# DaveStrickland/AstroPhotography

Measured on AMD Instinct MI355X. Metric: Mpixels/sec calibrate+sigma-clip-stack, higher is better.
Workload: dtype f32; 1 GPU; C2: 64x4096x4096 f32 per GPU, fused bias/dark/flat + 3-sigma maxiters-5 median-centred clipped mean; frames_per_gpu=64, frames_total=64, height=4096, width=4096, parallelism=single GPU

## Files before the change

### astrophotography_amd/csrc/stack_calibrate.h

```cpp
#pragma once
#include "stack_sort.h"

namespace apgpu_stack {

using namespace apgpu;

struct StackParams {
    const void *frames;
    const float *bias, *dark, *nflat, *exp_ratio, *pedestal;
    const uint8_t *pixmask;
    float *mean, *median, *std;
    void *moments;
    int32_t *count;
    int64_t P;
    int64_t stride;
    double sl2, su2;
    int N;
    int still_biased;
    int center;
    int dev;
    int maxiters;
    int moments64;
    double *mean64, *std64;
    int single_kernel;
// ... 90 lines not shown
    }
}

template <int NP>
__device__ __forceinline__ void stage_commit(const StackParams &prm, FrameScalars<NP> &fs, float e, float ped)
{
    const int t = threadIdx.x;
    if (t < NP) {
        fs.e[t] = e;
        fs.ped[t] = ped;
        fs.pad[t] = t < prm.N ? -__builtin_inff() : __builtin_inff();
    }
    __syncthreads();
}

template <int NP>
__device__ __forceinline__ void stage_frame_scalars(const StackParams &prm, FrameScalars<NP> &fs)
{
    for (int t = threadIdx.x; t < NP; t += blockDim.x) {
        const int ff = t < prm.N ? t : prm.N - 1;
        fs.e[t] = prm.exp_ratio ? prm.exp_ratio[ff] : 0.f;
        fs.ped[t] = prm.pedestal ? prm.pedestal[ff] : 0.f;
        fs.pad[t] = t < prm.N ? -__builtin_inff() : __builtin_inff();
    }
    __syncthreads();
}

#ifndef APGPU_PIN_RAGGED_F32
#define APGPU_PIN_RAGGED_F32 0
#endif
template <int NP, typename RawT, bool FULL, int F0 = 0, int CNT = NP, int MINN = 0, int NSTATIC = 0>
__device__ __forceinline__ void load_raw(const StackParams &prm, int64_t base, int lane, RawT (&raw)[CNT])
{
    const RawT *fb = static_cast<const RawT *>(prm.frames) + base + (int64_t)F0 * prm.stride;
    int nframes = NSTATIC > 0 ? NSTATIC : prm.N;
    if constexpr (!FULL && NSTATIC == 0) asm volatile("" : "+s"(nframes));
#pragma unroll
    for (int f = 0; f < CNT; f++) {
        constexpr bool SKIP = !FULL && MINN < NP;
        if (!SKIP || F0 + f < MINN || F0 + f < nframes) raw[f] = fb[lane];
        else raw[f] = RawT(0);
        if (FULL || (SKIP && F0 + f + 1 < MINN) || F0 + f + 1 < nframes) fb += prm.stride;
        if ((f & 7) == 7) __builtin_amdgcn_sched_barrier(0);
    }
    if constexpr ((sizeof(RawT) == 2 || APGPU_PIN_RAGGED_F32) && !FULL && MINN < NP && NSTATIC == 0) {
#pragma unroll
        for (int f = 0; f < CNT; f++) asm volatile("" : "+v"(raw[f]));
    }
}

typedef float v2f __attribute__((ext_vector_type(2)));

template <int NP, typename RawT, bool HAS_PED, int F0 = 0, int CNT = NP, bool RANGE_GUARD = true, int MINN = NP, bool UNI_E = false,
          bool E_DIRECT = false>
__device__ __forceinline__ bool calibrate_fast(const FrameScalars<NP> &fs, const RawT (&raw)[CNT], float b, float D, float nf,
                                               bool dodiv, float (&v)[NP], int nframes = NP, int plo = 0, const float *eg = nullptr)
{
    const float nfe = dodiv ? nf : 1.0f;
    const float y = __fdiv_rn(1.0f, nfe);
    const float yl = recip_low(nfe, y);
    const float anf = fabsf(nfe);
    const bool nf_ok = (anf >= 0x1p-40f && anf <= 0x1p40f);
    float mx = 0.f, mn = __builtin_inff();
    if constexpr (NP >= 2) {
        v2f acc = {0.f, 0.f};
        const v2f b2 = {b, b}, D2 = {D, D}, nf2 = {-nfe, -nfe}, y2 = {y, y}, yl2 = {yl, yl}, zero2 = {0.f, 0.f};
        float e0 = 0.f;
        if constexpr (UNI_E) {
            if constexpr (E_DIRECT) e0 = ((const float __attribute__((address_space(4))) *)(uintptr_t)eg)[0];
            else e0 = fs.e[0];
        }
        const float ds0 = e0 * D;
        const v2f ds_uni = {ds0, ds0};
#pragma unroll
        for (int g = 0; g < CNT; g += 2) {
            const int f = F0 + g;
            if ((f & ~7) >= MINN && (f & ~7) >= nframes) continue;
            v2f x = {to_f32(raw[g]), to_f32(raw[g + 1])};
            if constexpr (HAS_PED) {
                const v2f ped = {fs.ped[f], fs.ped[f + 1]};
                x = x + ped;
            }
            x = x - b2;
            v2f ds = ds_uni;
            if constexpr (UNI_E) {
            } else if constexpr (E_DIRECT) {
                typedef const float __attribute__((address_space(4))) cfloat;
                const cfloat *ec = (const cfloat *)(uintptr_t)eg;
                const int f0 = (f < MINN || f < nframes) ? f : nframes - 1;
                const int f1 = (f + 1 < MINN || f + 1 < nframes) ? f + 1 : nframes - 1;
                const v2f e2 = {ec[f0], ec[f1]};
                ds = e2 * D2;
            } else {
                const v2f e2 = {fs.e[f], fs.e[f + 1]};
                ds = e2 * D2;
            }
            x = x - ds;
            const v2f q0 = __builtin_elementwise_fma(x, y2, x * yl2);
            const v2f r0 = __builtin_elementwise_fma(nf2, q0, x);
            const v2f q = __builtin_elementwise_fma(r0, y2, q0);
            v[f] = q.x;
            v[f + 1] = q.y;
            acc = __builtin_elementwise_fma(q, zero2, acc);
            if constexpr (RANGE_GUARD) {
                mx = fmaxf(fmaxf(mx, fabsf(q.x)), fabsf(q.y));
                mn = fminf(fminf(mn, fabsf(q.x)), fabsf(q.y));
            }
        }
        if constexpr (MINN < NP) {
#pragma unroll
            for (int g = 0; g < CNT; g++)
                if (F0 + g >= MINN && F0 + g >= nframes)
                    v[F0 + g] = (F0 + g < nframes + plo) ? -__builtin_inff() : __builtin_inff();
        }
        const bool range_ok = !RANGE_GUARD || !dodiv || (mx < 0x1p50f && mn > 0x1p-50f);
        return nf_ok && range_ok && (acc.x == 0.f) && (acc.y == 0.f);
    } else {
        float x = to_f32(raw[0]);
        if constexpr (HAS_PED) x = x + fs.ped[0];
        x = x - b;
        const float ds = (E_DIRECT ? eg[0] : fs.e[0]) * D;
        x = x - ds;
        const float q = div_by_recip(x, nfe, y, yl);
        v[0] = q;
        const float acc = __builtin_fmaf(q, 0.0f, 0.0f);
        const bool range_ok = !dodiv || (fabsf(q) < 0x1p50f && fabsf(q) > 0x1p-50f);
        return nf_ok && range_ok && (acc == 0.f);
    }
}

template <int LO, int NP>
__device__ __forceinline__ float uniform_pick(const float (&v)[NP], int idx)
{
    if constexpr (LO >= NP - 1) return v[NP - 1];
    else {
        if (idx <= LO) return v[LO];
        return uniform_pick<LO + 1, NP>(v, idx);
    }
}

template <int NP, int MINN = NP>
__device__ __forceinline__ bool range_ok_sorted(const float (&v)[NP], bool dodiv, int nvalid = NP, int plo = 0)
{
    float lo = v[0];
    float hi;
    if constexpr (MINN >= NP) hi = v[NP - 1];
    else {
        if (plo > 0) lo = uniform_pick<0, NP>(v, plo);
        hi = uniform_pick<(MINN > 0 ? MINN - 1 : 0), NP>(v, plo + __builtin_amdgcn_readfirstlane(nvalid) - 1);
    }
    const bool big_ok = fmaxf(fabsf(lo), fabsf(hi)) < 0x1p50f;
    const bool one_sign = lo > 0x1p-50f || hi < -0x1p-50f;
    bool small_ok = one_sign;
    if (wave_any(dodiv && !one_sign)) {
        float mn = __builtin_inff();
        if constexpr (NP >= 2) {
#pragma unroll
            for (int i = 0; i < NP; i += 2) mn = fminf(fminf(mn, fabsf(v[i])), fabsf(v[i + 1]));
        } else {
            mn = fabsf(v[0]);
        }
        small_ok = mn > 0x1p-50f;
    }
    return !dodiv || (big_ok && small_ok);
}

template <int NP, typename RawT>
struct EarlyLoads {
    RawT raw[NP];
    float b, d, nf;
    bool skip;
};

template <int NP, typename RawT, bool CALIB, bool FULL, int MINN, int NSTATIC = 0>
__device__ __forceinline__ void issue_early_loads(const StackParams &prm, int64_t base, int lane, EarlyLoads<NP, RawT> &L)
{
    const int64_t p = base + lane;
    L.b = 0.f; L.d = 0.f; L.nf = 1.f;
    if constexpr (CALIB) {
        L.b = prm.bias[p];
        L.d = prm.dark[p];
        if (prm.nflat) L.nf = prm.nflat[p];
    }
    L.skip = prm.pixmask && prm.pixmask[p];
    __builtin_amdgcn_sched_barrier(0);
    load_raw<NP, RawT, FULL, 0, NP, MINN, NSTATIC>(prm, base, lane, L.raw);
}

template <int NP>
__device__ __forceinline__ bool exposures_uniform(const FrameScalars<NP> &fs)
{
    bool same = true;
    for (int t = threadIdx.x & 63; t < NP; t += 64) same = same && (fs.e[t] == fs.e[0]);
    return wave_all(same);
}

template <int NP>
__device__ __forceinline__ bool ratios_uniform(const float *eg, int nframes)
{
    typedef const float __attribute__((address_space(4))) cfloat;
    const cfloat *ec = (const cfloat *)(uintptr_t)eg;
    const int e0 = __builtin_amdgcn_readfirstlane(__float_as_int(ec[0]));
    bool same = true;
#pragma unroll
    for (int f = 1; f < NP; f++) same = same && (f >= nframes || __builtin_amdgcn_readfirstlane(__float_as_int(ec[f < nframes ? f : 0])) == e0);
    return same;
}

struct ColumnCtx {
    float b, D, nf;
    bool dodiv, skip;
    bool range_pending;
};

template <int NP, typename RawT, bool CALIB, bool FINITE_ONLY, bool FULL, int NRAW>
__device__ __forceinline__ int load_column_exact(const StackParams &prm, const FrameScalars<NP> &fs, int64_t p, const ColumnCtx &cx,
                                                 const RawT (&raw)[NRAW], float (&v)[NP], int plo = 0)
{
    const int N = prm.N;
    int n = 0;
    const RawT *fp = static_cast<const RawT *>(prm.frames) + p;
    int nleft = N;
    asm volatile("" : "+s"(nleft));
#pragma unroll
    for (int f = 0; f < NP; f++) {
        float x;
        if constexpr (CALIB) {
            x = to_f32(*fp);
            if (FULL || f + 1 < nleft) fp += prm.stride;
        } else {
            x = to_f32(raw[f < NRAW ? f : 0]);
        }
        if constexpr (CALIB) {
            typedef const float __attribute__((address_space(4))) cfloat;
            const int ff = (FULL || f < N) ? f : N - 1;
            const float e = prm.exp_ratio ? ((const cfloat *)(uintptr_t)prm.exp_ratio)[ff] : 0.f;
            const float ped = prm.pedestal ? ((const cfloat *)(uintptr_t)prm.pedestal)[ff] : 0.f;
            if (ped != 0.f) x = x + ped;
            x = x - cx.b;
            const float ds = e * cx.D;
            x = x - ds;
            if (cx.dodiv) x = __fdiv_rn(x, cx.nf);
        }
        bool ok;
        if constexpr (FINITE_ONLY) ok = fabsf(x) < __builtin_inff();
        else ok = (x == x);
        ok = ok && (FULL || f < N) && !cx.skip;
        n += ok ? 1 : 0;
        v[f] = ok ? x : __builtin_inff();
        if (!FULL && f >= N && f < N + plo) v[f] = -__builtin_inff();
    }
    return n;
}

template <int NP, typename RawT, bool CALIB, bool FINITE_ONLY, bool FULL, int MINN = padded_minn(NP, FULL), bool FORCE_HALVES = false, bool PRE = false>
__device__ __forceinline__ int load_column(const StackParams &prm, const FrameScalars<NP> &fs, int64_t base, int lane,
                                           float (&v)[NP], ColumnCtx &cx, int plo = 0, const EarlyLoads<NP, RawT> &pre = EarlyLoads<NP, RawT>())
{
    const int N = prm.N;
// ... 125 lines not shown
```

### astrophotography_amd/csrc/stack_kernels.h

```cpp
#pragma once
#include "stack_reduce.h"

namespace apgpu_stack {

using namespace apgpu;

#ifndef APGPU_LEAN_MIN_BLOCKS
#define APGPU_LEAN_MIN_BLOCKS 3
#endif
#ifndef APGPU_PLUS_MIN_BLOCKS
#define APGPU_PLUS_MIN_BLOCKS 3
#endif
#ifndef APGPU_WIDE_MIN_BLOCKS
#define APGPU_WIDE_MIN_BLOCKS 2
#endif
#ifndef APGPU_PADDED_MIN_BLOCKS
#define APGPU_PADDED_MIN_BLOCKS 3
#endif

constexpr int kRedoSegs = 256;
constexpr int kWsLine = 16;
constexpr int kWsStats = kRedoSegs * kWsLine;
constexpr int kWsCall = kWsStats + 16;
constexpr int kWsMadCount = 8, kWsMadMode = 10, kMadSample = 16;
// ... 322 lines not shown
#pragma unroll
                for (int i = 0; i < NP; i++) {
                    if (i >= nslots) continue;
                    const double dd = widen(v[i]) - mean64;
                    const bool in = (i >= T && i < NP - T) || ((i >= a) && (i < b));
                    const double d = in ? dd : 0.0;
                    q1 = fma(d, d, q1);
                }
                if (good) ko->std[p] = (float)sqrt(q1 > 0.0 ? q1 / (double)(b - a) : 0.0);
            }
        }
    }
}

template <int NP, typename RawT, bool CALIB, bool FULL = true, int PADS = 0, bool PLUS = false>
__global__ __launch_bounds__(256, NP <= 64 ? APGPU_FAST_MIN_BLOCKS : ((FULL || PADS > 0 || NP <= 96) ? 3 : 2)) void stack_fast_kernel(const StackParams prm)
{
    static_assert(PADS == 0 || (!FULL && PADS <= NP - prev_slots(NP)), "static pads: a padded stack");
    constexpr int MINN = fast_kernel_minn(NP, FULL);
    constexpr int PLO = PADS > 0 ? (PADS >> 1) : -1, PHI = PADS > 0 ? PADS - (PADS >> 1) : -1;
    static_assert(fast_kernel_slots(NP), "the fast kernel is the float32 fast path");
    static_assert(CALIB || sizeof(RawT) == 4, "unfused stacks: float32 frames");
    constexpr int T = !CALIB ? (NP >= 20 ? 8 : 6) : fast_kernel_tail(NP, FULL);
    constexpr bool HALVES = CALIB && NP >= 104;
    const int64_t base = (int64_t)blockIdx.x * 256;
    const int lane = threadIdx.x;
    const int64_t p = base + lane;
    __shared__ FrameScalars<NP> fs;
    const int N = FULL ? NP : (PADS > 0 ? NP - PADS : prm.N);
    const int plo = FULL ? 0 : (NP - N) >> 1, phi = FULL ? 0 : NP - N - plo;
    const bool alert = fast_kernel_alert();
    if (fast_block_bails<256>(alert, prm.redo)) {
        give_blocks_up<256>();
        return;
    }
    bool good = false;
    if (base + 256 <= prm.P) {
        float v[NP];
        bool dodiv = false;
        int nonfin = 0;
        if constexpr (HALVES) {
            constexpr int HN = NP / 2, NS = PADS > 0 ? NP - PADS : 0;
            const float b = prm.bias[p];
            const float D = prm.still_biased ? prm.dark[p] - b : prm.dark[p];
            float nf = 1.f;
            if (prm.nflat) {
                nf = prm.nflat[p];
                dodiv = (nf != 0.f);
            }
            good = !(prm.pixmask && prm.pixmask[p]);
            __builtin_amdgcn_sched_barrier(0);
            RawT half[HN];
            load_raw<NP, RawT, FULL, 0, HN, MINN, NS>(prm, base, lane, half);
            good = calibrate_fast<NP, RawT, false, 0, HN, false, MINN, false, true>(fs, half, b, D, nf, dodiv, v, N, plo, prm.exp_ratio) && good;
            load_raw<NP, RawT, FULL, HN, HN, MINN, NS>(prm, base, lane, half);
            good = calibrate_fast<NP, RawT, false, HN, HN, false, MINN, false, true>(fs, half, b, D, nf, dodiv, v, N, plo, prm.exp_ratio) && good;
        }
        EarlyLoads<NP, RawT> L;
        if constexpr (!HALVES) {
            issue_early_loads<NP, RawT, CALIB, FULL, MINN, (PADS > 0 ? NP - PADS : 0)>(prm, base, lane, L);
            good = !L.skip;
        }
        if constexpr (HALVES) {
        } else if constexpr (CALIB) {
            const float b = L.b;
            const float D = prm.still_biased ? L.d - b : L.d;
            float nf = 1.f;
            if (prm.nflat) {
                nf = L.nf;
                dodiv = (nf != 0.f);
            }
            good = calibrate_fast<NP, RawT, false, 0, NP, false, MINN, false, true>(fs, L.raw, b, D, nf, dodiv, v, N, plo, prm.exp_ratio) && good;
        } else {
#pragma unroll
            for (int f = 0; f < NP; f++) {
                if (FULL || f < MINN || f < N) {
                    const float x = L.raw[f];
                    v[f] = fabsf(x) < __builtin_inff() ? x : __builtin_inff();
                } else {
                    v[f] = (f < N + plo) ? -__builtin_inff() : __builtin_inff();
                }
            }
        }
#ifdef APGPU_VARIANT_STRIP
        if (wave_any(good)) {
            if (APGPU_VARIANT_STRIP == 1) {
                sort_column<NP, T>(v);
                if constexpr (CALIB) good = good && range_ok_sorted<NP, MINN>(v, dodiv, N, plo);
            }
            float acc[4] = {good ? 0.f : 1.f, 0.f, 0.f, 0.f};
#pragma unroll
            for (int i = 0; i < NP; i++) acc[i & 3] += v[i];
            if (prm.mean) prm.mean[p] = (acc[0] + acc[1]) + (acc[2] + acc[3]);
        }
        __shared__ char geometry[40 * 1024];
        if (prm.N < 0) geometry[lane] = 1;
        return;
#endif
        if (wave_any(good)) {
            sort_column<NP, T>(v);
            if constexpr (CALIB) good = good && range_ok_sorted<NP, MINN>(v, dodiv, N, plo);
            else {
#pragma unroll
                for (int k = 1; k <= T; k++) nonfin += (v[NP - k] == __builtin_inff()) ? 1 : 0;
                good = good && nonfin < T;
            }
            if (wave_any(good)) finish_fast_column<NP, T, CALIB, PLO, PHI, PLUS>(v, good, p, plo, CALIB ? phi : nonfin);
        }
    }
    fast_blocks_done<256>(alert, prm.redo);
    redo_push(!good && p < late_params()->P, p, alert);
}

template <int NP, typename RawT, bool CALIB, bool FULL>
__global__ __launch_bounds__(256) void stack_median_kernel(const StackParams prm)
{
    const int64_t base = (int64_t)blockIdx.x * blockDim.x;
    const int lane = threadIdx.x;
    const int64_t p = base + lane;
    __shared__ FrameScalars<NP> fs;
    if (needs_staging<CALIB, FULL, NP>(prm)) stage_frame_scalars<NP>(prm, fs);
    if (p >= prm.P) return;
    float v[NP];
    const int n = load_sorted_column<NP, RawT, CALIB, false, FULL>(prm, fs, base, lane, v);
    const float m1 = pick_at<NP>(v, (n - 1) >> 1);
    const float m2 = pick_at<NP>(v, n >> 1);
    const double med = ((double)m1 + (double)m2) / 2.0;
    if (prm.median) prm.median[p] = n > 0 ? (float)med : __builtin_nanf("");
    if (prm.count) prm.count[p] = n;
}

template <bool CALIB>
__device__ __forceinline__ float calibrate_exact_u16(unsigned raw, float b, float D, float e, float nf, bool dodiv)
{
    float x = (float)raw;
    if constexpr (CALIB) {
        x = x - b;
        const float ds = e * D;
        x = x - ds;
        if (dodiv) x = __fdiv_rn(x, nf);
    }
    return x;
}

template <int NP, bool CALIB, bool FULL>
__global__ __launch_bounds__(256) void stack_median_u16_kernel(const StackParams prm)
{
    __shared__ FrameScalars<NP> fs;
    const int lane = threadIdx.x;
    bool monotone = true;
    if constexpr (CALIB) {
        stage_frame_scalars<NP>(prm, fs);
        const bool differs = lane < NP && (!(fs.e[lane] == fs.e[0]) || fs.ped[lane] != 0.f);
        monotone = !__syncthreads_or(differs);
    } else if constexpr (!FULL) {
        stage_frame_scalars<NP>(prm, fs);
    }
    const int N = prm.N;
    if (monotone) {
        const int64_t p2 = ((int64_t)blockIdx.x * 256 + lane) * 2;
        if (p2 >= prm.P) return;
// ... 32 lines not shown
                nn[0] = n2.x; nn[1] = n2.y;
                dodiv[0] = n2.x != 0.f;
                dodiv[1] = n2.y != 0.f;
            }
        }
        float med[2];
        int cnt[2];
#pragma unroll
        for (int h = 0; h < 2; h++) {
            const unsigned r1 = (m1 >> (16 * h)) & 0xffffu, r2 = (m2 >> (16 * h)) & 0xffffu;
            const float c1 = calibrate_exact_u16<CALIB>(r1, bb[h], dd[h], e, nn[h], dodiv[h]);
            const float c2 = calibrate_exact_u16<CALIB>(r2, bb[h], dd[h], e, nn[h], dodiv[h]);
            const bool skip = prm.pixmask && prm.pixmask[p2 + h];
            const bool any = (c1 == c1) && (c2 == c2) && !skip;
            cnt[h] = any ? N : 0;
            med[h] = any ? (float)(((double)c1 + (double)c2) / 2.0) : __builtin_nanf("");
        }
        if (prm.median) *reinterpret_cast<float2 *>(prm.median + p2) = make_float2(med[0], med[1]);
        if (prm.count) *reinterpret_cast<int2 *>(prm.count + p2) = make_int2(cnt[0], cnt[1]);
    } else {
#pragma unroll 1
        for (int half = 0; half < 2; half++) {
            const int64_t base = ((int64_t)blockIdx.x * 2 + half) * 256;
            const int64_t p = base + lane;
            if (p >= prm.P) break;
            float v[NP];
            StackParams q = prm;
            asm volatile("" : "+s"(q.N));
            const int n = load_sorted_column<NP, uint16_t, CALIB, false, FULL, NP>(q, fs, base, lane, v);
            const float m1 = pick_at<NP>(v, (n - 1) >> 1);
            const float m2 = pick_at<NP>(v, n >> 1);
            const double med = ((double)m1 + (double)m2) / 2.0;
            if (prm.median) prm.median[p] = n > 0 ? (float)med : __builtin_nanf("");
            if (prm.count) prm.count[p] = n;
        }
    }
}

template <int NP, bool CALIB, bool FULL, int T, int MINN, int PLO = -1, int PHI = -1>
__device__ __forceinline__ bool fast_raw_column(const FrameScalars<NP> &fs, const uint32_t (&cur)[NP / 2], float b, float D, float nf,
                                                bool dv, bool masked, const float *eg, int64_t p, int N, int plo, int phi)
{
    float v[NP];
    bool good = !masked;
    {
        float rawf[NP];
#pragma unroll
        for (int k = 0; k < NP / 2; k++) {
            rawf[2 * k] = (float)(cur[k] & 0xffffu);
            rawf[2 * k + 1] = (float)(cur[k] >> 16);
        }
        if constexpr (CALIB) {
            const bool increasing = (fabsf(b) < __builtin_inff()) && (fabsf(D) < __builtin_inff()) && (!dv || (nf > 0.f && nf < __builtin_inff()));
            good = calibrate_fast<NP, float, false, 0, NP, false, NP, true, true>(fs, rawf, b, D, nf, dv, v, NP, 0, eg) && increasing && good;
        } else {
#pragma unroll
            for (int f = 0; f < NP; f++) v[f] = rawf[f];
        }
    }
    if constexpr (!FULL) {
#pragma unroll
        for (int i = 0; i < NP; i++) {
            if (i < NP - MINN && i < plo) v[i] = -__builtin_inff();
            if (i >= MINN && i >= NP - phi) v[i] = __builtin_inff();
        }
    }
    if constexpr (CALIB) good = good && range_ok_sorted<NP, (MINN < NP ? MINN : 0)>(v, dv, N, plo);
    if (wave_any(good)) finish_fast_column<NP, T, true, PLO, PHI>(v, good, p, plo, phi);
    return good;
}

constexpr bool pairs_padded_slots(int np) { return fast32_possible_padded(np, padded_minn(np, false)) || np == 104; }

template <int NP, bool CALIB, bool FULL, int PADS = 0>
__global__ __launch_bounds__(256, NP <= 80 ? APGPU_FAST_MIN_BLOCKS : (NP <= 104 ? 3 : 2)) void stack_fast_u16_pairs_kernel(const StackParams prm)
{
    static_assert(PADS == 0 || (!FULL && PADS <= NP - padded_minn(NP, false)), "static pads: a padded stack");
    constexpr int MINN = padded_minn(NP, FULL);
    constexpr int PLO = PADS > 0 ? (PADS >> 1) : -1, PHI = PADS > 0 ? PADS - (PADS >> 1) : -1;
    static_assert(FULL ? fast_kernel_slots(NP) : pairs_padded_slots(NP), "the fast kernel is the float32 fast path");
    constexpr int T = FULL ? kFastTail : fast_tail_padded(NP);
    constexpr int HP = NP / 2;
    __shared__ uint32_t parked[HP][256];
    __shared__ FrameScalars<NP> fs;
    const int lane = threadIdx.x;
    const int N = FULL ? NP : (PADS > 0 ? NP - PADS : prm.N);
    const int plo = FULL ? 0 : (NP - N) >> 1, phi = FULL ? 0 : NP - N - plo;
    const int64_t p2 = ((int64_t)blockIdx.x * 256 + lane) * 2;
    bool good0 = false, good1 = false;
    const bool tile_ok = ((int64_t)blockIdx.x + 1) * 512 <= prm.P;
    const bool alert = fast_kernel_alert();
    bool give_up = fast_block_bails<512>(alert, prm.redo);
    if constexpr (CALIB) give_up = give_up || !ratios_uniform<NP>(prm.exp_ratio, N);
    if (give_up) {
        give_blocks_up<512>();
        return;
    }
    if (tile_ok) {
        float bb[2] = {0.f, 0.f}, dd[2] = {0.f, 0.f}, nn[2] = {1.f, 1.f};
        bool dodiv[2] = {false, false};
        bool skip[2] = {false, false};
        if constexpr (CALIB) {
            const float2 b2 = *reinterpret_cast<const float2 *>(prm.bias + p2);
            const float2 d2 = *reinterpret_cast<const float2 *>(prm.dark + p2);
            bb[0] = b2.x; bb[1] = b2.y;
            dd[0] = prm.still_biased ? d2.x - b2.x : d2.x;
            dd[1] = prm.still_biased ? d2.y - b2.y : d2.y;
            if (prm.nflat) {
                const float2 n2 = *reinterpret_cast<const float2 *>(prm.nflat + p2);
                nn[0] = n2.x; nn[1] = n2.y;
                dodiv[0] = n2.x != 0.f;
                dodiv[1] = n2.y != 0.f;
            }
        }
        if (prm.pixmask) {
            skip[0] = prm.pixmask[p2] != 0;
            skip[1] = prm.pixmask[p2 + 1] != 0;
        }
        __builtin_amdgcn_sched_barrier(0);
        uint32_t w[NP];
// ... 280 lines not shown
```

### astrophotography_amd/csrc/stack_sort.h

```cpp
#pragma once
#include "common.h"

#include <utility>

namespace apgpu_stack {

using namespace apgpu;


#ifdef APGPU_PROFILE_SECTIONS
#define APGPU_MARK(name) do { __builtin_amdgcn_sched_barrier(0); asm volatile("; APGPU_SECTION " name); __builtin_amdgcn_sched_barrier(0); } while (0)
#else
#define APGPU_MARK(name) asm volatile("; APGPU_SECTION " name)
#endif

__device__ __forceinline__ bool wave_any(bool p) { return __builtin_amdgcn_ballot_w64(p) != 0; }
__device__ __forceinline__ bool wave_all(bool p) { return __builtin_amdgcn_ballot_w64(!p) == 0; }

struct CE {
    unsigned char a, b;
};

template <int NP>
struct Net {
// ... 24 lines not shown
                        net.ce[c].b = (unsigned char)(i + j + k);
                        c++;
                    }
            }
    net.n = c;
    return net;
}

template <int NP, int P0, int T>
constexpr Net<NP> make_pruned_net()
{
    constexpr Net<NP> full = make_net<NP, P0>();
    bool live[NP] = {};
    for (int i = 0; i < T; i++) live[i] = live[NP - 1 - i] = true;
    for (int i = (NP - T - 1) / 2; i <= (NP + T) / 2; i++) live[i] = true;
    bool keep[NP * 12 + 1] = {};
    for (int c = full.n - 1; c >= 0; c--) {
        const int a = full.ce[c].a, b = full.ce[c].b;
        if (live[a] || live[b]) {
            keep[c] = true;
            live[a] = live[b] = true;
        }
    }
    Net<NP> net{};
    int n = 0;
    for (int c = 0; c < full.n; c++)
        if (keep[c]) net.ce[n++] = full.ce[c];
    net.n = n;
    return net;
}

template <int NP, int P0, int LO, int HI>
constexpr Net<NP> make_window_net()
{
    constexpr Net<NP> full = make_net<NP, P0>();
    bool live[NP] = {};
    for (int i = LO; i < HI; i++) live[i] = true;
    bool keep[NP * 12 + 1] = {};
    for (int c = full.n - 1; c >= 0; c--) {
        const int a = full.ce[c].a, b = full.ce[c].b;
        if (live[a] || live[b]) {
            keep[c] = true;
            live[a] = live[b] = true;
        }
    }
    Net<NP> net{};
    int n = 0;
    for (int c = 0; c < full.n; c++)
        if (keep[c]) net.ce[n++] = full.ce[c];
    net.n = n;
    return net;
}

__device__ __forceinline__ void cmpx(float &x, float &y)
{
    float lo, hi;
    asm("v_min_f32 %0, %1, %2" : "=v"(lo) : "v"(x), "v"(y));
    asm("v_max_f32 %0, %1, %2" : "=v"(hi) : "v"(x), "v"(y));
    x = lo;
    y = hi;
}

__device__ __forceinline__ void sort4(float &a, float &b, float &c, float &d)
{
    float x0, x1, x2, o0, o1, o2, o3;
    asm("v_min3_f32 %0, %1, %2, %3" : "=v"(x0) : "v"(a), "v"(b), "v"(c));
    asm("v_med3_f32 %0, %1, %2, %3" : "=v"(x1) : "v"(a), "v"(b), "v"(c));
    asm("v_max3_f32 %0, %1, %2, %3" : "=v"(x2) : "v"(a), "v"(b), "v"(c));
    asm("v_min_f32 %0, %1, %2" : "=v"(o0) : "v"(x0), "v"(d));
    asm("v_med3_f32 %0, %1, %2, %3" : "=v"(o1) : "v"(x0), "v"(x1), "v"(d));
    asm("v_med3_f32 %0, %1, %2, %3" : "=v"(o2) : "v"(x1), "v"(x2), "v"(d));
    asm("v_max_f32 %0, %1, %2" : "=v"(o3) : "v"(x2), "v"(d));
    a = o0;
    b = o1;
    c = o2;
    d = o3;
}

template <int NP, int P0, int T, int BASE, int... I>
__device__ __forceinline__ void net_chunk(float (&v)[NP], std::integer_sequence<int, I...>)
{
    constexpr Net<NP> net = T > 0 ? make_pruned_net<NP, P0, (T > 0 ? T : 1)>() : make_net<NP, P0>();
    (cmpx(v[net.ce[BASE + I].a], v[net.ce[BASE + I].b]), ...);
}

template <int NP, int P0, int T, int BASE>
__device__ __forceinline__ void net_from(float (&v)[NP])
{
    constexpr int total = T > 0 ? make_pruned_net<NP, P0, (T > 0 ? T : 1)>().n : make_net<NP, P0>().n;
    constexpr int CH = 64;
    if constexpr (BASE < total) {
        constexpr int len = (total - BASE < CH) ? total - BASE : CH;
        net_chunk<NP, P0, T, BASE>(v, std::make_integer_sequence<int, len>{});
        net_from<NP, P0, T, BASE + len>(v);
    }
}

template <int NP, int P0, int LO, int HI, int BASE, int... I>
__device__ __forceinline__ void window_net_chunk(float (&v)[NP], std::integer_sequence<int, I...>)
{
    constexpr Net<NP> net = make_window_net<NP, P0, LO, HI>();
    (cmpx(v[net.ce[BASE + I].a], v[net.ce[BASE + I].b]), ...);
}

template <int NP, int P0, int LO, int HI, int BASE = 0>
__device__ __forceinline__ void window_net_from(float (&v)[NP])
{
    constexpr int total = make_window_net<NP, P0, LO, HI>().n;
    constexpr int CH = 64;
    if constexpr (BASE < total) {
        constexpr int len = (total - BASE < CH) ? total - BASE : CH;
        window_net_chunk<NP, P0, LO, HI, BASE>(v, std::make_integer_sequence<int, len>{});
        window_net_from<NP, P0, LO, HI, BASE + len>(v);
    }
}

struct NetOp {
    unsigned char w[4];
    unsigned char k;
    unsigned char stage;
};

template <int NP>
struct OpNet {
    NetOp op[NP * 9 + 24];
    int n;
};

constexpr NetOp kSort16Ops[18] = {
    {{0, 1, 2, 3}, 4},    {{4, 5, 6, 7}, 4},    {{8, 9, 10, 11}, 4},  {{12, 13, 14, 15}, 4},
    {{0, 4, 8, 12}, 4},   {{1, 5, 9, 13}, 4},   {{2, 6, 10, 14}, 4},  {{3, 7, 11, 15}, 4},
    {{3, 5, 12, 0}, 3},   {{7, 10, 13, 0}, 3},  {{5, 6, 9, 0}, 3},    {{2, 5, 8, 0}, 3},   {{1, 2, 4, 0}, 3},
    {{7, 9, 12, 0}, 3},   {{11, 13, 14, 0}, 3}, {{6, 7, 8, 0}, 3},    {{10, 11, 12, 0}, 3}, {{3, 4, 5, 0}, 3}};
constexpr NetOp kSort8Ops[8] = {{{0, 1, 2, 0}, 3}, {{3, 4, 5, 0}, 3}, {{0, 6, 7, 0}, 3}, {{1, 4, 6, 0}, 3},
                                {{2, 5, 7, 0}, 3}, {{0, 1, 3, 0}, 3}, {{2, 3, 4, 0}, 3}, {{4, 5, 6, 0}, 3}};
constexpr NetOp kMerge16Ops[] = {
    {{9, 23, 0, 0}, 2}, {{8, 22, 0, 0}, 2}, {{7, 21, 0, 0}, 2}, {{10, 24, 0, 0}, 2}, {{6, 20, 0, 0}, 2}, {{11, 25, 0, 0}, 2},
    {{5, 19, 0, 0}, 2}, {{12, 26, 0, 0}, 2}, {{4, 12, 18, 0}, 3}, {{13, 19, 27, 0}, 3}, {{3, 17, 0, 0}, 2}, {{14, 20, 28, 0}, 3},
    {{15, 21, 29, 0}, 3}, {{2, 10, 16, 0}, 3}, {{7, 11, 17, 0}, 3}, {{1, 9, 13, 0}, 3}, {{0, 8, 12, 0}, 3}, {{18, 22, 30, 0}, 3},
    {{19, 23, 31, 0}, 3}, {{20, 24, 0, 0}, 2}, {{14, 16, 18, 0}, 3}, {{13, 15, 17, 0}, 3}, {{21, 23, 25, 0}, 3}, {{24, 26, 30, 0}, 3},
    {{6, 8, 10, 0}, 3}, {{1, 3, 5, 0}, 3}, {{0, 4, 6, 0}, 3}, {{25, 27, 31, 0}, 3}, {{5, 6, 7, 0}, 3}, {{15, 17, 19, 0}, 3},
    {{19, 20, 22, 0}, 3}, {{12, 14, 16, 0}, 3}, {{9, 11, 12, 0}, 3}, {{27, 28, 30, 0}, 3}, {{0, 1, 2, 0}, 3}, {{29, 30, 31, 0}, 3},
    {{13, 14, 0, 0}, 2}, {{7, 8, 0, 0}, 2}, {{21, 22, 0, 0}, 2}, {{23, 24, 0, 0}, 2}, {{25, 26, 0, 0}, 2}, {{17, 18, 0, 0}, 2},
    {{9, 10, 0, 0}, 2}, {{15, 16, 0, 0}, 2}, {{3, 4, 0, 0}, 2}};

template <int NP>
constexpr void add_op(OpNet<NP> &net, const NetOp &o, int off, int stage)
// ... 8 lines not shown
        net.op[net.n++] = r;
    }
}

template <int NP, int T>
constexpr OpNet<NP> make_opnet()
{
    OpNet<NP> net{};
    net.n = 0;
    for (int base = 0; base < NP; base += 16) {
        if (NP - base <= 8) {
            for (const NetOp &o : kSort8Ops) add_op<NP>(net, o, base, 0);
        } else {
            for (const NetOp &o : kSort16Ops) add_op<NP>(net, o, base, 0);
        }
    }
    for (int base = 0; base + 16 < NP; base += 32)
        for (const NetOp &o : kMerge16Ops) add_op<NP>(net, o, base, 1);
    constexpr int P2 = next_pow2(NP);
    for (int p = 32; p < P2; p *= 2)
        for (int k = p; k >= 1; k /= 2)
            for (int j = k % p; j <= P2 - 1 - k; j += 2 * k) {
                const int lim = (k - 1 < P2 - j - k - 1) ? k - 1 : P2 - j - k - 1;
                for (int i = 0; i <= lim; i++)
                    if ((i + j) / (p * 2) == (i + j + k) / (p * 2)) {
                        const NetOp ce = {{(unsigned char)(i + j), (unsigned char)(i + j + k), 0, 0}, 2, 2};
                        add_op<NP>(net, ce, 0, 2);
                    }
            }
    if (T > 0) {
        bool live[NP] = {};
        for (int i = 0; i < T; i++) live[i] = live[NP - 1 - i] = true;
        for (int i = (NP - T - 1) / 2; i <= (NP + T) / 2; i++) live[i] = true;
        bool keep[NP * 9 + 24] = {};
        for (int c = net.n - 1; c >= 0; c--) {
            bool any = false;
            for (int i = 0; i < net.op[c].k; i++) any = any || live[net.op[c].w[i]];
            if (any) {
                keep[c] = true;
                for (int i = 0; i < net.op[c].k; i++) live[net.op[c].w[i]] = true;
            }
        }
        int n = 0;
        for (int c = 0; c < net.n; c++)
            if (keep[c]) net.op[n++] = net.op[c];
        net.n = n;
    }
    return net;
}

template <int NP, int T>
inline constexpr OpNet<NP> kOpNet = make_opnet<NP, T>();

__device__ __forceinline__ void sort3(float &a, float &b, float &c)
{
    float x0, x1, x2;
    asm("v_min3_f32 %0, %1, %2, %3" : "=v"(x0) : "v"(a), "v"(b), "v"(c));
    asm("v_med3_f32 %0, %1, %2, %3" : "=v"(x1) : "v"(a), "v"(b), "v"(c));
    asm("v_max3_f32 %0, %1, %2, %3" : "=v"(x2) : "v"(a), "v"(b), "v"(c));
    a = x0;
    b = x1;
    c = x2;
}

template <int NP, int T, int I>
__device__ __forceinline__ void opnet_apply(float (&v)[NP])
{
    constexpr NetOp o = kOpNet<NP, T>.op[I];
    if constexpr (o.k == 2) cmpx(v[o.w[0]], v[o.w[1]]);
    else if constexpr (o.k == 3) sort3(v[o.w[0]], v[o.w[1]], v[o.w[2]]);
    else sort4(v[o.w[0]], v[o.w[1]], v[o.w[2]], v[o.w[3]]);
}

template <int NP, int T, int BASE, int... I>
__device__ __forceinline__ void opnet_chunk(float (&v)[NP], std::integer_sequence<int, I...>)
{
    (opnet_apply<NP, T, BASE + I>(v), ...);
}

template <int NP, int T, int BASE = 0>
__device__ __forceinline__ void opnet_from(float (&v)[NP])
{
    constexpr int total = kOpNet<NP, T>.n;
    constexpr int CH = 64;
    if constexpr (BASE < total) {
        constexpr int len = (total - BASE < CH) ? total - BASE : CH;
        opnet_chunk<NP, T, BASE>(v, std::make_integer_sequence<int, len>{});
        opnet_from<NP, T, BASE + len>(v);
    }
}

template <int NP, int PRUNE_T = 0>
__device__ __forceinline__ void sort_column(float (&v)[NP])
{
#ifndef APGPU_VARIANT_BATCHER_ONLY
    if constexpr (NP >= 8 && NP % 4 == 0) {
        opnet_from<NP, PRUNE_T>(v);
    } else
#endif
    if constexpr (NP >= 4 && NP % 4 == 0) {
#pragma unroll
        for (int g = 0; g < NP; g += 4) sort4(v[g], v[g + 1], v[g + 2], v[g + 3]);
        net_from<NP, 4, PRUNE_T, 0>(v);
    } else if constexpr (NP > 1) {
        net_from<NP, 1, PRUNE_T, 0>(v);
    }
}

template <int LO, int LEN, int NP>
__device__ __forceinline__ float pick_rel(const float (&v)[NP], int rel)
{
    if constexpr (LEN == 1) {
        return v[LO];
    } else if constexpr ((LEN & (LEN - 1)) == 0) {
        constexpr int H = LEN / 2;
        float lo = pick_rel<LO, H, NP>(v, rel);
        float hi = pick_rel<LO + H, H, NP>(v, rel);
        return (rel & H) ? hi : lo;
    } else {
        constexpr int H = next_pow2(LEN) / 2;
        float lo = pick_rel<LO, H, NP>(v, rel);
        float hi = pick_rel<LO + H, LEN - H, NP>(v, rel - H);
        return (rel >= H) ? hi : lo;
    }
}

template <int NP>
__device__ __forceinline__ float pick_at(const float (&v)[NP], int idx)
{
    idx = idx < 0 ? 0 : (idx > NP - 1 ? NP - 1 : idx);
    return pick_rel<0, NP, NP>(v, idx);
}

template <int K, int NP>
__device__ __forceinline__ void pick_window(const float (&v)[NP], int k, int i1, int i2, float &m1, float &m2)
{
    if (k == K) {
        m1 = pick_rel<4 * K, 8, NP>(v, i1 - 4 * K);
        m2 = pick_rel<4 * K, 8, NP>(v, i2 - 4 * K);
    } else if constexpr (4 * (K + 1) + 8 <= NP) {
        pick_window<K + 1, NP>(v, k, i1, i2, m1, m2);
    }
}

template <int NP>
__device__ __forceinline__ void pick_middle(const float (&v)[NP], int i1, int i2, float &m1, float &m2)
{
    if constexpr (NP <= 8) {
        m1 = pick_at<NP>(v, i1);
        m2 = pick_at<NP>(v, i2);
    } else {
        constexpr int WLO = NP / 2 - 4;
        const bool inside = (i1 >= WLO) && (i2 < WLO + 8);
        if (wave_all(inside)) {
            m1 = pick_rel<WLO, 8, NP>(v, i1 - WLO);
            m2 = pick_rel<WLO, 8, NP>(v, i2 - WLO);
        } else {
            int k = (__builtin_amdgcn_readfirstlane(i1) - 2) >> 2;
// ... 79 lines not shown
```

Baseline: 1.258 million Mpixels/s.

## Defer non-finite detection to NaN-propagating sort maxima instead of per-frame FMA accumulator

Drops the per-frame fma(q,0,acc) finiteness accumulator in calibration. In its place, the sorting network uses v_maximum3_f32, which propagates NaN, so non-finite values reach the top of the sorted column. The sorted-range check then catches them. It also specialises the calibrate path on uniform exposure ratios, which keeps the dark-scale multiply scalar, and simplifies the ratio-uniformity check to an XOR-reduce. It risks mis-ordering or missed detection if NaN handling in the sort network differs from the old semantics, and the new lambda dispatch increases code size.

```diff
diff --git a/astrophotography_amd/csrc/stack_calibrate.h b/astrophotography_amd/csrc/stack_calibrate.h
--- a/astrophotography_amd/csrc/stack_calibrate.h
+++ b/astrophotography_amd/csrc/stack_calibrate.h
@@ -166,7 +166,7 @@
 typedef float v2f __attribute__((ext_vector_type(2)));
 
 template <int NP, typename RawT, bool HAS_PED, int F0 = 0, int CNT = NP, bool RANGE_GUARD = true, int MINN = NP, bool UNI_E = false,
-          bool E_DIRECT = false>
+          bool E_DIRECT = false, bool FINITE_LATER = false>
 __device__ __forceinline__ bool calibrate_fast(const FrameScalars<NP> &fs, const RawT (&raw)[CNT], float b, float D, float nf,
                                                bool dodiv, float (&v)[NP], int nframes = NP, int plo = 0, const float *eg = nullptr)
 {
@@ -215,7 +215,7 @@
             const v2f q = __builtin_elementwise_fma(r0, y2, q0);
             v[f] = q.x;
             v[f + 1] = q.y;
-            acc = __builtin_elementwise_fma(q, zero2, acc);
+            if constexpr (!FINITE_LATER) acc = __builtin_elementwise_fma(q, zero2, acc);
             if constexpr (RANGE_GUARD) {
                 mx = fmaxf(fmaxf(mx, fabsf(q.x)), fabsf(q.y));
                 mn = fminf(fminf(mn, fabsf(q.x)), fabsf(q.y));
@@ -228,7 +228,8 @@
                     v[F0 + g] = (F0 + g < nframes + plo) ? -__builtin_inff() : __builtin_inff();
         }
         const bool range_ok = !RANGE_GUARD || !dodiv || (mx < 0x1p50f && mn > 0x1p-50f);
-        return nf_ok && range_ok && (acc.x == 0.f) && (acc.y == 0.f);
+        if constexpr (FINITE_LATER) return nf_ok && range_ok;
+        else return nf_ok && range_ok && (acc.x == 0.f) && (acc.y == 0.f);
     } else {
         float x = to_f32(raw[0]);
         if constexpr (HAS_PED) x = x + fs.ped[0];
@@ -253,7 +254,7 @@
     }
 }
 
-template <int NP, int MINN = NP>
+template <int NP, int MINN = NP, bool FINITE = false>
 __device__ __forceinline__ bool range_ok_sorted(const float (&v)[NP], bool dodiv, int nvalid = NP, int plo = 0)
 {
     float lo = v[0];
@@ -263,7 +264,15 @@
         if (plo > 0) lo = uniform_pick<0, NP>(v, plo);
         hi = uniform_pick<(MINN > 0 ? MINN - 1 : 0), NP>(v, plo + __builtin_amdgcn_readfirstlane(nvalid) - 1);
     }
-    const bool big_ok = fmaxf(fabsf(lo), fabsf(hi)) < 0x1p50f;
+    bool big_ok;
+    if constexpr (FINITE) {
+        float m;
+        asm("v_maximum3_f32 %0, |%1|, |%2|, |%2|" : "=v"(m) : "v"(lo), "v"(hi));
+        big_ok = m < 0x1p50f || (!dodiv && m < __builtin_inff());
+        if constexpr (MINN < NP) big_ok = big_ok && (v[NP - 1] == v[NP - 1]);
+    } else {
+        big_ok = fmaxf(fabsf(lo), fabsf(hi)) < 0x1p50f;
+    }
     const bool one_sign = lo > 0x1p-50f || hi < -0x1p-50f;
     bool small_ok = one_sign;
     if (wave_any(dodiv && !one_sign)) {
@@ -276,7 +285,8 @@
         }
         small_ok = mn > 0x1p-50f;
     }
-    return !dodiv || (big_ok && small_ok);
+    if constexpr (FINITE) return big_ok && (!dodiv || small_ok);
+    else return !dodiv || (big_ok && small_ok);
 }
 
 template <int NP, typename RawT>
@@ -315,10 +325,10 @@
     typedef const float __attribute__((address_space(4))) cfloat;
     const cfloat *ec = (const cfloat *)(uintptr_t)eg;
     const int e0 = __builtin_amdgcn_readfirstlane(__float_as_int(ec[0]));
-    bool same = true;
-#pragma unroll
-    for (int f = 1; f < NP; f++) same = same && (f >= nframes || __builtin_amdgcn_readfirstlane(__float_as_int(ec[f < nframes ? f : 0])) == e0);
-    return same;
+    int diff = 0;
+#pragma unroll
+    for (int f = 1; f < NP; f++) diff |= __builtin_amdgcn_readfirstlane(__float_as_int(ec[f < nframes ? f : 0])) ^ e0;
+    return diff == 0;
 }
 
 struct ColumnCtx {
diff --git a/astrophotography_amd/csrc/stack_kernels.h b/astrophotography_amd/csrc/stack_kernels.h
--- a/astrophotography_amd/csrc/stack_kernels.h
+++ b/astrophotography_amd/csrc/stack_kernels.h
@@ -398,61 +398,73 @@
             __builtin_amdgcn_sched_barrier(0);
             RawT half[HN];
             load_raw<NP, RawT, FULL, 0, HN, MINN, NS>(prm, base, lane, half);
-            good = calibrate_fast<NP, RawT, false, 0, HN, false, MINN, false, true>(fs, half, b, D, nf, dodiv, v, N, plo, prm.exp_ratio) && good;
+            good = calibrate_fast<NP, RawT, false, 0, HN, false, MINN, false, true, true>(fs, half, b, D, nf, dodiv, v, N, plo, prm.exp_ratio) && good;
             load_raw<NP, RawT, FULL, HN, HN, MINN, NS>(prm, base, lane, half);
-            good = calibrate_fast<NP, RawT, false, HN, HN, false, MINN, false, true>(fs, half, b, D, nf, dodiv, v, N, plo, prm.exp_ratio) && good;
-        }
-        EarlyLoads<NP, RawT> L;
-        if constexpr (!HALVES) {
-            issue_early_loads<NP, RawT, CALIB, FULL, MINN, (PADS > 0 ? NP - PADS : 0)>(prm, base, lane, L);
-            good = !L.skip;
-        }
-        if constexpr (HALVES) {
-        } else if constexpr (CALIB) {
-            const float b = L.b;
-            const float D = prm.still_biased ? L.d - b : L.d;
-            float nf = 1.f;
-            if (prm.nflat) {
-                nf = L.nf;
-                dodiv = (nf != 0.f);
-            }
-            good = calibrate_fast<NP, RawT, false, 0, NP, false, MINN, false, true>(fs, L.raw, b, D, nf, dodiv, v, N, plo, prm.exp_ratio) && good;
+            good = calibrate_fast<NP, RawT, false, HN, HN, false, MINN, false, true, true>(fs, half, b, D, nf, dodiv, v, N, plo, prm.exp_ratio) && good;
+        }
+        auto rest = [&](auto uni_c) {
+            constexpr bool UNI = decltype(uni_c)::value;
+            EarlyLoads<NP, RawT> L;
+            if constexpr (!HALVES) {
+                issue_early_loads<NP, RawT, CALIB, FULL, MINN, (PADS > 0 ? NP - PADS : 0)>(prm, base, lane, L);
+                good = !L.skip;
+            }
+            if constexpr (HALVES) {
+            } else if constexpr (CALIB) {
+                const float b = L.b;
+                const float D = prm.still_biased ? L.d - b : L.d;
+                float nf = 1.f;
+                if (prm.nflat) {
+                    nf = L.nf;
+                    dodiv = (nf != 0.f);
+                }
+                good = calibrate_fast<NP, RawT, false, 0, NP, false, MINN, UNI, true, true>(fs, L.raw, b, D, nf, dodiv, v, N, plo, prm.exp_ratio) && good;
+            } else {
+#pragma unroll
+                for (int f = 0; f < NP; f++) {
+                    if (FULL || f < MINN || f < N) {
+                        const float x = L.raw[f];
+                        v[f] = fabsf(x) < __builtin_inff() ? x : __builtin_inff();
+                    } else {
+                        v[f] = (f < N + plo) ? -__builtin_inff() : __builtin_inff();
+                    }
+                }
+            }
+#ifdef APGPU_VARIANT_STRIP
+            if (wave_any(good)) {
+                if (APGPU_VARIANT_STRIP == 1) {
+                    sort_column<NP, T, CALIB>(v);
+                    if constexpr (CALIB) good = good && range_ok_sorted<NP, MINN, true>(v, dodiv, N, plo);
+                }
+                float acc[4] = {good ? 0.f : 1.f, 0.f, 0.f, 0.f};
+#pragma unroll
+                for (int i = 0; i < NP; i++) acc[i & 3] += v[i];
+                if (prm.mean) prm.mean[p] = (acc[0] + acc[1]) + (acc[2] + acc[3]);
+            }
+            return;
+#endif
+            if (wave_any(good)) {
+                sort_column<NP, T, CALIB>(v);
+                if constexpr (CALIB) good = good && range_ok_sorted<NP, MINN, true>(v, dodiv, N, plo);
+                else {
+#pragma unroll
+                    for (int k = 1; k <= T; k++) nonfin += (v[NP - k] == __builtin_inff()) ? 1 : 0;
+                    good = good && nonfin < T;
+                }
+                if (wave_any(good)) finish_fast_column<NP, T, CALIB, PLO, PHI, PLUS>(v, good, p, plo, CALIB ? phi : nonfin);
+            }
+        };
+        if constexpr (CALIB && !HALVES) {
+            if (ratios_uniform<NP>(prm.exp_ratio, N)) rest(std::true_type{});
+            else rest(std::false_type{});
         } else {
-#pragma unroll
-            for (int f = 0; f < NP; f++) {
-                if (FULL || f < MINN || f < N) {
-                    const float x = L.raw[f];
-                    v[f] = fabsf(x) < __builtin_inff() ? x : __builtin_inff();
-                } else {
-                    v[f] = (f < N + plo) ? -__builtin_inff() : __builtin_inff();
-                }
-            }
+            rest(std::false_type{});
         }
 #ifdef APGPU_VARIANT_STRIP
-        if (wave_any(good)) {
-            if (APGPU_VARIANT_STRIP == 1) {
-                sort_column<NP, T>(v);
-                if constexpr (CALIB) good = good && range_ok_sorted<NP, MINN>(v, dodiv, N, plo);
-            }
-            float acc[4] = {good ? 0.f : 1.f, 0.f, 0.f, 0.f};
-#pragma unroll
-            for (int i = 0; i < NP; i++) acc[i & 3] += v[i];
-            if (prm.mean) prm.mean[p] = (acc[0] + acc[1]) + (acc[2] + acc[3]);
-        }
         __shared__ char geometry[40 * 1024];
         if (prm.N < 0) geometry[lane] = 1;
         return;
 #endif
-        if (wave_any(good)) {
-            sort_column<NP, T>(v);
-            if constexpr (CALIB) good = good && range_ok_sorted<NP, MINN>(v, dodiv, N, plo);
-            else {
-#pragma unroll
-                for (int k = 1; k <= T; k++) nonfin += (v[NP - k] == __builtin_inff()) ? 1 : 0;
-                good = good && nonfin < T;
-            }
-            if (wave_any(good)) finish_fast_column<NP, T, CALIB, PLO, PHI, PLUS>(v, good, p, plo, CALIB ? phi : nonfin);
-        }
     }
     fast_blocks_done<256>(alert, prm.redo);
     redo_push(!good && p < late_params()->P, p, alert);
@@ -591,7 +603,7 @@
         }
         if constexpr (CALIB) {
             const bool increasing = (fabsf(b) < __builtin_inff()) && (fabsf(D) < __builtin_inff()) && (!dv || (nf > 0.f && nf < __builtin_inff()));
-            good = calibrate_fast<NP, float, false, 0, NP, false, NP, true, true>(fs, rawf, b, D, nf, dv, v, NP, 0, eg) && increasing && good;
+            good = calibrate_fast<NP, float, false, 0, NP, false, NP, true, true, true>(fs, rawf, b, D, nf, dv, v, NP, 0, eg) && increasing && good;
         } else {
 #pragma unroll
             for (int f = 0; f < NP; f++) v[f] = rawf[f];
@@ -604,7 +616,7 @@
             if (i >= MINN && i >= NP - phi) v[i] = __builtin_inff();
         }
     }
-    if constexpr (CALIB) good = good && range_ok_sorted<NP, (MINN < NP ? MINN : 0)>(v, dv, N, plo);
+    if constexpr (CALIB) good = good && range_ok_sorted<NP, (MINN < NP ? MINN : 0), true>(v, dv, N, plo);
     if (wave_any(good)) finish_fast_column<NP, T, true, PLO, PHI>(v, good, p, plo, phi);
     return good;
 }
diff --git a/astrophotography_amd/csrc/stack_sort.h b/astrophotography_amd/csrc/stack_sort.h
--- a/astrophotography_amd/csrc/stack_sort.h
+++ b/astrophotography_amd/csrc/stack_sort.h
@@ -100,47 +100,74 @@
     return net;
 }
 
+__device__ __forceinline__ float max2(float x, float y, std::false_type)
+{
+    float hi;
+    asm("v_max_f32 %0, %1, %2" : "=v"(hi) : "v"(x), "v"(y));
+    return hi;
+}
+__device__ __forceinline__ float max2(float x, float y, std::true_type)
+{
+    float hi;
+    asm("v_maximum3_f32 %0, %1, %2, %2" : "=v"(hi) : "v"(x), "v"(y));
+    return hi;
+}
+__device__ __forceinline__ float max3(float x, float y, float z, std::false_type)
+{
+    float hi;
+    asm("v_max3_f32 %0, %1, %2, %3" : "=v"(hi) : "v"(x), "v"(y), "v"(z));
+    return hi;
+}
+__device__ __forceinline__ float max3(float x, float y, float z, std::true_type)
+{
+    float hi;
+    asm("v_maximum3_f32 %0, %1, %2, %3" : "=v"(hi) : "v"(x), "v"(y), "v"(z));
+    return hi;
+}
+
+template <bool NANMAX = false>
 __device__ __forceinline__ void cmpx(float &x, float &y)
 {
-    float lo, hi;
+    float lo;
     asm("v_min_f32 %0, %1, %2" : "=v"(lo) : "v"(x), "v"(y));
-    asm("v_max_f32 %0, %1, %2" : "=v"(hi) : "v"(x), "v"(y));
+    const float hi = max2(x, y, std::bool_constant<NANMAX>{});
     x = lo;
     y = hi;
 }
 
+template <bool NANMAX = false>
 __device__ __forceinline__ void sort4(float &a, float &b, float &c, float &d)
 {
-    float x0, x1, x2, o0, o1, o2, o3;
+    float x0, x1, o0, o1, o2;
     asm("v_min3_f32 %0, %1, %2, %3" : "=v"(x0) : "v"(a), "v"(b), "v"(c));
     asm("v_med3_f32 %0, %1, %2, %3" : "=v"(x1) : "v"(a), "v"(b), "v"(c));
-    asm("v_max3_f32 %0, %1, %2, %3" : "=v"(x2) : "v"(a), "v"(b), "v"(c));
+    const float x2 = max3(a, b, c, std::bool_constant<NANMAX>{});
     asm("v_min_f32 %0, %1, %2" : "=v"(o0) : "v"(x0), "v"(d));
     asm("v_med3_f32 %0, %1, %2, %3" : "=v"(o1) : "v"(x0), "v"(x1), "v"(d));
     asm("v_med3_f32 %0, %1, %2, %3" : "=v"(o2) : "v"(x1), "v"(x2), "v"(d));
-    asm("v_max_f32 %0, %1, %2" : "=v"(o3) : "v"(x2), "v"(d));
+    const float o3 = max2(x2, d, std::bool_constant<NANMAX>{});
     a = o0;
     b = o1;
     c = o2;
     d = o3;
 }
 
-template <int NP, int P0, int T, int BASE, int... I>
+template <int NP, int P0, int T, int BASE, bool NANMAX, int... I>
 __device__ __forceinline__ void net_chunk(float (&v)[NP], std::integer_sequence<int, I...>)
 {
     constexpr Net<NP> net = T > 0 ? make_pruned_net<NP, P0, (T > 0 ? T : 1)>() : make_net<NP, P0>();
-    (cmpx(v[net.ce[BASE + I].a], v[net.ce[BASE + I].b]), ...);
-}
-
-template <int NP, int P0, int T, int BASE>
+    (cmpx<NANMAX>(v[net.ce[BASE + I].a], v[net.ce[BASE + I].b]), ...);
+}
+
+template <int NP, int P0, int T, int BASE, bool NANMAX = false>
 __device__ __forceinline__ void net_from(float (&v)[NP])
 {
     constexpr int total = T > 0 ? make_pruned_net<NP, P0, (T > 0 ? T : 1)>().n : make_net<NP, P0>().n;
     constexpr int CH = 64;
     if constexpr (BASE < total) {
         constexpr int len = (total - BASE < CH) ? total - BASE : CH;
-        net_chunk<NP, P0, T, BASE>(v, std::make_integer_sequence<int, len>{});
-        net_from<NP, P0, T, BASE + len>(v);
+        net_chunk<NP, P0, T, BASE, NANMAX>(v, std::make_integer_sequence<int, len>{});
+        net_from<NP, P0, T, BASE + len, NANMAX>(v);
     }
 }
 
@@ -255,58 +282,59 @@
 template <int NP, int T>
 inline constexpr OpNet<NP> kOpNet = make_opnet<NP, T>();
 
+template <bool NANMAX = false>
 __device__ __forceinline__ void sort3(float &a, float &b, float &c)
 {
-    float x0, x1, x2;
+    float x0, x1;
     asm("v_min3_f32 %0, %1, %2, %3" : "=v"(x0) : "v"(a), "v"(b), "v"(c));
     asm("v_med3_f32 %0, %1, %2, %3" : "=v"(x1) : "v"(a), "v"(b), "v"(c));
-    asm("v_max3_f32 %0, %1, %2, %3" : "=v"(x2) : "v"(a), "v"(b), "v"(c));
+    const float x2 = max3(a, b, c, std::bool_constant<NANMAX>{});
     a = x0;
     b = x1;
     c = x2;
 }
 
-template <int NP, int T, int I>
+template <int NP, int T, int I, bool NANMAX>
 __device__ __forceinline__ void opnet_apply(float (&v)[NP])
 {
     constexpr NetOp o = kOpNet<NP, T>.op[I];
-    if constexpr (o.k == 2) cmpx(v[o.w[0]], v[o.w[1]]);
-    else if constexpr (o.k == 3) sort3(v[o.w[0]], v[o.w[1]], v[o.w[2]]);
-    else sort4(v[o.w[0]], v[o.w[1]], v[o.w[2]], v[o.w[3]]);
-}
-
-template <int NP, int T, int BASE, int... I>
+    if constexpr (o.k == 2) cmpx<NANMAX>(v[o.w[0]], v[o.w[1]]);
+    else if constexpr (o.k == 3) sort3<NANMAX>(v[o.w[0]], v[o.w[1]], v[o.w[2]]);
+    else sort4<NANMAX>(v[o.w[0]], v[o.w[1]], v[o.w[2]], v[o.w[3]]);
+}
+
+template <int NP, int T, int BASE, bool NANMAX, int... I>
 __device__ __forceinline__ void opnet_chunk(float (&v)[NP], std::integer_sequence<int, I...>)
 {
-    (opnet_apply<NP, T, BASE + I>(v), ...);
-}
-
-template <int NP, int T, int BASE = 0>
+    (opnet_apply<NP, T, BASE + I, NANMAX>(v), ...);
+}
+
+template <int NP, int T, int BASE = 0, bool NANMAX = false>
 __device__ __forceinline__ void opnet_from(float (&v)[NP])
 {
     constexpr int total = kOpNet<NP, T>.n;
     constexpr int CH = 64;
     if constexpr (BASE < total) {
         constexpr int len = (total - BASE < CH) ? total - BASE : CH;
-        opnet_chunk<NP, T, BASE>(v, std::make_integer_sequence<int, len>{});
-        opnet_from<NP, T, BASE + len>(v);
-    }
-}
-
-template <int NP, int PRUNE_T = 0>
+        opnet_chunk<NP, T, BASE, NANMAX>(v, std::make_integer_sequence<int, len>{});
+        opnet_from<NP, T, BASE + len, NANMAX>(v);
+    }
+}
+
+template <int NP, int PRUNE_T = 0, bool NANMAX = false>
 __device__ __forceinline__ void sort_column(float (&v)[NP])
 {
 #ifndef APGPU_VARIANT_BATCHER_ONLY
     if constexpr (NP >= 8 && NP % 4 == 0) {
-        opnet_from<NP, PRUNE_T>(v);
+        opnet_from<NP, PRUNE_T, 0, NANMAX>(v);
     } else
 #endif
     if constexpr (NP >= 4 && NP % 4 == 0) {
 #pragma unroll
-        for (int g = 0; g < NP; g += 4) sort4(v[g], v[g + 1], v[g + 2], v[g + 3]);
-        net_from<NP, 4, PRUNE_T, 0>(v);
+        for (int g = 0; g < NP; g += 4) sort4<NANMAX>(v[g], v[g + 1], v[g + 2], v[g + 3]);
+        net_from<NP, 4, PRUNE_T, 0, NANMAX>(v);
     } else if constexpr (NP > 1) {
-        net_from<NP, 1, PRUNE_T, 0>(v);
+        net_from<NP, 1, PRUNE_T, 0, NANMAX>(v);
     }
 }
 
```

Result: faster. 1.284 million Mpixels/s (median of 6 runs) (+2.1%).
